# scraed/LanPaint

Measured on AMD Instinct MI355X. Metric: langevin_think_iterations_per_sec, higher is better.
Workload: dtype f32; 1 GPU; c2_sdxl: latent 1x4x128x128 per GPU, 30 sigmas x 5 think iterations, 50% box mask, stub backbone x->(0.9x,0.8x), VE/Karras schedule; rng=torch, graph=auto, mask_format=f32, mask_seen_by_kernels=bits, captured_calls=1, backbone_io=f32, replicas=1, rows_per_gpu=1, global_rows=1, latent_elements_per_gpu=65536

## Files before the change

lanpaint_amd/csrc/aux_kernels.hip:

```cpp
#include "lp_common.h"

namespace lp {

__global__ void lp_coeffs_kernel(lp_hyper h, const float* __restrict__ ve, int ve_stride,
                                 const float* __restrict__ abt, int abt_stride, const float* __restrict__ rs,
                                 int rs_stride, const float* __restrict__ step_ov, int step_stride,
                                 const float* __restrict__ t_model, int t_stride, int rows, float* __restrict__ table) {
    const int t = blockIdx.x * blockDim.x + threadIdx.x;
    const int r = t >> 2;
    if (r >= rows) return;
    const float abt_f = abt[static_cast<int64_t>(r) * abt_stride];
    const float ve_f = ve ? ve[static_cast<int64_t>(r) * ve_stride] : 0.0f;
    const float rs_f = rs ? rs[static_cast<int64_t>(r) * rs_stride] : 0.0f;
    const float tm_f = t_model ? t_model[static_cast<int64_t>(r) * t_stride] : 0.0f;
    const float oma = 1.0f - abt_f;
    const float step = step_ov ? step_ov[static_cast<int64_t>(r) * step_stride]
                               : h.step_size * fmaxf(oma, h.min_step_frac);
    coeffs_lane(h, abt_f, ve_f, rs_f, tm_f, step, (t >> 1) & 1, t & 1, table + static_cast<int64_t>(r) * LP_COEF_STRIDE);
}

__global__ void lp_sigma_times_kernel(const float* __restrict__ sigma, int rows, const float* __restrict__ schedule,
                                      int schedule_len, int is_flow, float* __restrict__ times,
                                      float* __restrict__ scalars, int32_t* __restrict__ seq_out, int32_t seq,
                                      const SigmaRule rule) {
    if (blockIdx.x != 0 || threadIdx.x >= kWave) return;
    sigma_rows_and_rule(sigma, rows, schedule, schedule_len, is_flow != 0, times, scalars, seq_out, seq, rule);
}

int sigma_times_rule_dispatch(const float* sigma, int rows, const float* schedule, int schedule_len, int is_flow,
                              float* times, float* scalars, int32_t* seq_out, int32_t seq, int32_t n_steps, int32_t early_stop,
                              int32_t total_steps, double min_step_frac, int32_t guess, uint64_t* valid_out, hipStream_t stream) {
    if (!sigma || !schedule || !times || !scalars || rows <= 0 || schedule_len <= 0) return LP_E_INVALID;
    const SigmaRule rule{n_steps, early_stop, total_steps, guess, min_step_frac, valid_out};
    hipLaunchKernelGGL(lp_sigma_times_kernel, dim3(1), dim3(64), 0, stream, sigma, rows, schedule, schedule_len, is_flow,
                       times, scalars, seq_out, seq, rule);
    return hipGetLastError() == hipSuccess ? LP_OK : LP_E_LAUNCH;
}

int sigma_times_dispatch(const float* sigma, int rows, const float* schedule, int schedule_len, int is_flow,
                         float* times, float* scalars, int32_t* seq_out, int32_t seq, hipStream_t stream) {
    return sigma_times_rule_dispatch(sigma, rows, schedule, schedule_len, is_flow, times, scalars, seq_out, seq, 0, 0, 0, 0.0, -1,
                                     nullptr, stream);
}

int coeffs_dispatch(const lp_hyper* h, const float* ve, int ve_stride, const float* abt, int abt_stride,
                    const float* rs, int rs_stride, const float* step_ov, int step_stride, const float* t_model,
                    int t_stride, int rows, float* table, hipStream_t stream) {
    if (!h || !abt || !table || rows <= 0) return LP_E_INVALID;
    if (!h->is_flow && !ve) return LP_E_INVALID;
    const int block = 64, lanes = rows * 4;
    hipLaunchKernelGGL(lp_coeffs_kernel, dim3((lanes + block - 1) / block), dim3(block), 0, stream, *h, ve, ve_stride,
                       abt, abt_stride, rs, rs_stride, step_ov, step_stride, t_model, t_stride, rows, table);
    return hipGetLastError() == hipSuccess ? LP_OK : LP_E_LAUNCH;
}

template <int VEC, int BLOCK>
__global__ __launch_bounds__(256) void lp_finalize_kernel(const void* a_mask, const void* a_model_out, const float* a_y,
                                                          const float* a_x_src, const uint64_t* a_io_table, int64_t a_n_el,
                                                          uint32_t a_flags, const lp_final_desc d_arg) {
    lp_final_desc d = d_arg;
    d.mask = a_mask; d.model_out = a_model_out; d.y = a_y; d.x_src = a_x_src; d.io_table = a_io_table;
    d.n_el = a_n_el; d.flags = a_flags;
    const int64_t groups = d.n_el / VEC;
    const int dt = x0_dtype(d.flags);
    const int64_t g = static_cast<int64_t>(blockIdx.x) * BLOCK + threadIdx.x;
    float* const x_dst = d.io_table ? reinterpret_cast<float*>(d.io_table[0]) : d.x_dst;
    float* const out = d.io_table ? reinterpret_cast<float*>(d.io_table[1]) : d.out;
    if (d.io_table && d.io_table[2] == 0ull) return;
    constexpr bool RA = VEC == 4 && BLOCK == 256;
    const bool in_range = g < groups;
    if (RA || in_range) {
        const int64_t i = (in_range ? g : groups - 1) * VEC;
        float m[VEC], mo[VEC], yv[VEC], o[VEC];
        Raw<VEC> m_raw, mo_raw, un_raw;
        load_mask_raw<VEC>(d.mask, d.flags, i, m_raw);
        float xs[VEC];
        bool need_mo = true, need_y = true;
        if constexpr (RA) {
            if (x_dst) load_f32<VEC>(d.x_src, i, xs);
            if ((d.flags & LP_FL_MASK_BITS) && !(d.flags & (LP_FL_CFG_FUSED | LP_FL_NO_REGION_SKIP))) {
                const uint32_t nib = (m_raw.w[0] >> (static_cast<uint32_t>(i) & 31u)) & 0xFu;
                need_y = __ballot(in_range && nib != 0u) != 0ull;
                need_mo = __ballot(in_range && nib != 0xFu) != 0ull;
            }
            if (!in_range) return;
        }
#pragma unroll
        for (int k = 0; k < VEC; ++k) mo_raw.w[k] = 0u, yv[k] = 0.0f;
        if (need_mo) load_raw<VEC>(d.model_out, dt, i, mo_raw);
        if (d.flags & LP_FL_CFG_FUSED) load_raw<VEC>(d.uncond, dt, i, un_raw);
        if (need_y) load_f32<VEC>(d.y, i, yv);
        if constexpr (!RA) {
            if (x_dst) load_f32<VEC>(d.x_src, i, xs);
        }
        cvt_mask<VEC>(d.flags, i, m_raw, m);
        cvt_raw<VEC>(dt, mo_raw, mo);
        if (d.flags & LP_FL_CFG_FUSED) {
            float un[VEC];
            cvt_raw<VEC>(dt, un_raw, un);
#pragma unroll
            for (int k = 0; k < VEC; ++k) mo[k] = un[k] + (mo[k] - un[k]) * d.cfg_scale;
        }
#pragma unroll
        for (int k = 0; k < VEC; ++k) o[k] = mo[k] * (1.0f - m[k]) + yv[k] * m[k];
        store_f32<VEC>(out, i, o);
        if (x_dst) store_f32<VEC>(x_dst, i, xs);
    }
    if (d.rng_bump_ptr && blockIdx.x == 0 && threadIdx.x == 0) *d.rng_bump_ptr += d.rng_bump;
}

static bool aligned(const void* p, size_t a) { return p == nullptr || (reinterpret_cast<uintptr_t>(p) % a) == 0; }

int finalize_dispatch(const lp_final_desc* dp, hipStream_t stream) {
    if (!dp) return LP_E_INVALID;
    const lp_final_desc& d = *dp;
    if (d.n_el <= 0 || !d.model_out || !d.y || !d.mask || (!d.out && !d.io_table)) return LP_E_INVALID;
    if ((d.x_dst || d.io_table) && !d.x_src) return LP_E_INVALID;
    if ((d.flags & LP_FL_CFG_FUSED) && !d.uncond) return LP_E_INVALID;
    if ((d.flags & LP_FL_MASK_BITS) && ((d.flags & (LP_FL_MASK_U8 | LP_FL_MASK_DENOISE)) || !aligned(d.mask, 4)))
        return LP_E_INVALID;
    const bool half = x0_dtype(d.flags) != DT_F32;
    const bool vec4 = (d.n_el % 4 == 0) && aligned(d.model_out, half ? 8 : 16) && aligned(d.uncond, half ? 8 : 16) &&
                      aligned(d.y, 16) &&
                      aligned(d.mask, (d.flags & (LP_FL_MASK_U8 | LP_FL_MASK_BITS)) ? 4 : 16) && aligned(d.x_src, 16) &&
                      (d.io_table ? true : (aligned(d.x_dst, 16) && aligned(d.out, 16)));
    const int vec = vec4 ? 4 : 1;
    const int64_t groups = d.n_el / vec;
    const int block = groups <= 64 * 1024 ? 64 : 256;
    const int64_t bx = (groups + block - 1) / block;
    if (bx > 0x7fffffff) return LP_E_INVALID;
#define LP_FINAL_ARGS d.mask, d.model_out, d.y, d.x_src, d.io_table, d.n_el, d.flags, d
    const dim3 grid(static_cast<unsigned>(bx));
    if (vec4 && block == 64) hipLaunchKernelGGL((lp_finalize_kernel<4, 64>), grid, dim3(64), 0, stream, LP_FINAL_ARGS);
    else if (vec4) hipLaunchKernelGGL((lp_finalize_kernel<4, 256>), grid, dim3(256), 0, stream, LP_FINAL_ARGS);
    else if (block == 64) hipLaunchKernelGGL((lp_finalize_kernel<1, 64>), grid, dim3(64), 0, stream, LP_FINAL_ARGS);
    else hipLaunchKernelGGL((lp_finalize_kernel<1, 256>), grid, dim3(256), 0, stream, LP_FINAL_ARGS);
#undef LP_FINAL_ARGS
    return hipGetLastError() == hipSuccess ? LP_OK : LP_E_LAUNCH;
}

__global__ __launch_bounds__(256) void lp_philox_kernel(float* __restrict__ out, int64_t n_el, uint64_t seed,
                                                        uint64_t offset, uint32_t slot) {
    for (int64_t e = static_cast<int64_t>(blockIdx.x) * blockDim.x + threadIdx.x; e < n_el;
         e += static_cast<int64_t>(gridDim.x) * blockDim.x) {
        float za, zb;
        normal_pair(static_cast<uint64_t>(e), offset, seed, za, zb);
        out[e] = slot ? zb : za;
    }
}

int philox_dispatch(float* out, int64_t n_el, uint64_t seed, uint64_t offset, uint32_t slot, hipStream_t stream) {
    if (!out || n_el <= 0) return LP_E_INVALID;
    if (slot > 1) return LP_E_INVALID;
    int64_t bx = (n_el + 255) / 256;
    if (bx > 4096) bx = 4096;
    hipLaunchKernelGGL(lp_philox_kernel, dim3(static_cast<unsigned>(bx)), dim3(256), 0, stream, out, n_el, seed,
                       offset, slot);
    return hipGetLastError() == hipSuccess ? LP_OK : LP_E_LAUNCH;
}

constexpr int kRingRows = 32, kRingCols = 62;

__global__ __launch_bounds__(256) void lp_ring_kernel(const float* __restrict__ mask, float* __restrict__ ring,
                                                      int height, int width) {
    __shared__ unsigned long long rowbits[kRingRows + 2];
    const int lane = threadIdx.x & (kWave - 1), wave = threadIdx.x / kWave;
    const int x0 = blockIdx.x * kRingCols - 1, y0 = blockIdx.y * kRingRows - 1;
    const int64_t plane = static_cast<int64_t>(blockIdx.z) * height * width;
    const int x = x0 + lane;
    const bool x_in = x >= 0 && x < width;

    for (int j = wave; j < kRingRows + 2; j += 4) {
        const int y = y0 + j;
        bool known = false;
        if (x_in && y >= 0 && y < height) known = mask[plane + static_cast<int64_t>(y) * width + x] > 0.5f;
        const unsigned long long bits = __ballot(known);
        if (lane == 0) rowbits[j] = bits;
    }
    __syncthreads();
    for (int j = 1 + wave; j <= kRingRows; j += 4) {
        const int y = y0 + j;
        if (y >= height) break;
        const unsigned long long k = rowbits[j];
        const unsigned long long nb = (k << 1) | (k >> 1) | rowbits[j - 1] | rowbits[j + 1];
        const unsigned long long rb = ~k & nb;
        if (lane >= 1 && lane <= kRingCols && x_in) {
            const int64_t idx = plane + static_cast<int64_t>(y) * width + x;
            ring[idx] = ((rb >> lane) & 1ull) ? (1.0f - mask[idx]) : 0.0f;
        }
    }
}

int ring_dispatch(const float* mask, float* ring, int64_t planes, int height, int width, hipStream_t stream) {
    if (!mask || !ring || planes <= 0 || height <= 0 || width <= 0) return LP_E_INVALID;
    if (planes > 65535) return LP_E_UNSUPPORTED;
    dim3 grid((width + kRingCols - 1) / kRingCols, (height + kRingRows - 1) / kRingRows, static_cast<unsigned>(planes));
    if (grid.y > 65535) return LP_E_UNSUPPORTED;
    hipLaunchKernelGGL(lp_ring_kernel, grid, dim3(256), 0, stream, mask, ring, height, width);
    return hipGetLastError() == hipSuccess ? LP_OK : LP_E_LAUNCH;
}

template <int V>
__global__ __launch_bounds__(256) void lp_wmse_partial_kernel(const float* __restrict__ a, const float* __restrict__ b,
                                                              const float* __restrict__ mask,
                                                              const float* __restrict__ ring, int64_t n_el,
                                                              double* __restrict__ scratch) {
    __shared__ double part[4][4];
    float s[4] = {0.f, 0.f, 0.f, 0.f};
    const int64_t groups = n_el / V;
    for (int64_t g = static_cast<int64_t>(blockIdx.x) * blockDim.x + threadIdx.x; g < groups;
         g += static_cast<int64_t>(gridDim.x) * blockDim.x) {
        float av[V], bv[V], mv[V], rv[V];
        load_f32<V>(a, g * V, av);
        load_f32<V>(b, g * V, bv);
        load_f32<V>(mask, g * V, mv);
        if (ring) load_f32<V>(ring, g * V, rv);
#pragma unroll
        for (int k = 0; k < V; ++k) {
            const float dv = av[k] - bv[k];
            const float d2 = dv * dv;
            const float w1 = 1.0f - mv[k];
            s[0] += d2 * w1;
            s[1] += w1;
            if (ring) {
                s[2] += d2 * rv[k];
                s[3] += rv[k];
            }
        }
    }
    double v[4] = {static_cast<double>(s[0]), static_cast<double>(s[1]), static_cast<double>(s[2]), static_cast<double>(s[3])};
    wave_sum_dpp(v);
    const int lane = threadIdx.x & (kWave - 1), wave = threadIdx.x / kWave;
    if (lane == kWave - 1) {
#pragma unroll
        for (int k = 0; k < 4; ++k) part[wave][k] = v[k];
    }
    __syncthreads();
    if (threadIdx.x < 4) {
        const int k = threadIdx.x;
        scratch[static_cast<int64_t>(blockIdx.x) * 4 + k] = part[0][k] + part[1][k] + part[2][k] + part[3][k];
    }
}

__global__ __launch_bounds__(64) void lp_wmse_final_kernel(const double* __restrict__ scratch, int blocks, double* __restrict__ acc) {
    double v[4] = {0.0, 0.0, 0.0, 0.0};
    for (int bidx = threadIdx.x; bidx < blocks; bidx += kWave) {
#pragma unroll
        for (int k = 0; k < 4; ++k) v[k] += scratch[static_cast<int64_t>(bidx) * 4 + k];
    }
    wave_sum_dpp(v);
    if (threadIdx.x == kWave - 1) {
#pragma unroll
        for (int k = 0; k < 4; ++k) acc[k] = v[k];
    }
}

int wmse_dispatch(const float* a, const float* b, const float* mask, const float* ring, int64_t n_el, double* acc,
                  double* scratch, int scratch_blocks, hipStream_t stream) {
    if (!a || !b || !mask || !acc || !scratch || n_el <= 0 || scratch_blocks <= 0) return LP_E_INVALID;
    const auto al16 = [](const void* p) { return (reinterpret_cast<uintptr_t>(p) & 15u) == 0; };
    const bool vec4 = n_el % 4 == 0 && al16(a) && al16(b) && al16(mask) && (!ring || al16(ring));
// ... 110 lines not shown
```

lanpaint_amd/csrc/lp_common.h:

```cpp
#pragma once
#include <hip/hip_runtime.h>
#include <hip/hip_ext.h>
#include <stdint.h>

#include "lanpaint_hip.h"

namespace lp {

constexpr int kWave = 64;

__device__ __forceinline__ int nearest_exact_index(int i, int in_size, int out_size, int rule) {
#pragma clang fp contract(off)
    const float scale = static_cast<float>(in_size) / static_cast<float>(out_size);
    const float at = static_cast<float>(i) + 0.5f;
    int s;
    if (rule == LP_NN_ATEN_SCALAR) {
        s = static_cast<int>(floorf(at * scale));
    } else {
        float src = (rule == LP_NN_ATEN_CPU_GENERIC_FMA) ? __builtin_fmaf(scale, at, -0.5f) : (scale * at - 0.5f);
        src = src < 0.0f ? 0.0f : src;
        s = static_cast<int>(floorf(static_cast<float>(static_cast<double>(src) + 0.5)));
    }
    return s < in_size - 1 ? s : in_size - 1;
}
// ... 241 lines not shown
            const u2 t = __builtin_nontemporal_load(reinterpret_cast<const u2*>(q));
            r.w[0] = t.x; r.w[1] = t.y;
        } else {
#pragma unroll
            for (int k = 0; k < V; ++k) r.w[k] = q[k];
        }
    }
}



template <int V>
__device__ __forceinline__ void cvt_raw(int dt, const Raw<V>& r, float (&o)[V]) {
    if (dt == DT_F32) {
#pragma unroll
        for (int k = 0; k < V; ++k) o[k] = __uint_as_float(r.w[k]);
    } else {
        uint16_t h[V];
        if constexpr (V == 4) {
            h[0] = r.w[0] & 0xffffu; h[1] = r.w[0] >> 16; h[2] = r.w[1] & 0xffffu; h[3] = r.w[1] >> 16;
        } else {
#pragma unroll
            for (int k = 0; k < V; ++k) h[k] = static_cast<uint16_t>(r.w[k]);
        }
#pragma unroll
        for (int k = 0; k < V; ++k) o[k] = (dt == DT_BF16) ? bf16_to_f32(h[k]) : f16_to_f32(h[k]);
    }
}

template <int V>
__device__ __forceinline__ void cvt_raw(int dt, const Raw<V>& r, float (&o)[V], int64_t) {
    cvt_raw<V>(dt, r, o);
}

template <int V, int W, typename IX>
__device__ __forceinline__ void load_raw_w(const void* __restrict__ p, int dt, const IX& i, Raw<V>& r) {
    if constexpr (W == 4) load_raw<V>(p, DT_F32, i, r);
    else if constexpr (W == 2) load_raw<V>(p, DT_BF16, i, r);
    else load_raw<V>(p, dt, i, r);
}

template <int V>
__device__ __forceinline__ void load_any(const void* __restrict__ p, int dt, int64_t i, float (&o)[V]) {
    Raw<V> r;
    load_raw<V>(p, dt, i, r);
    cvt_raw<V>(dt, r, o);
}


template <int V>
__device__ __forceinline__ void store_any(void* __restrict__ p, int dt, int64_t i, const float (&v)[V]) {
    if (dt == DT_F32) {
        store_f32<V>(static_cast<float*>(p), i, v);
    } else {
        uint16_t* q = static_cast<uint16_t*>(p) + i;
        if constexpr (V == 4) {
            u2 t;
            t.x = pack_half2(dt, v[0], v[1]); t.y = pack_half2(dt, v[2], v[3]);
            __builtin_nontemporal_store(t, reinterpret_cast<u2*>(q));
        } else {
#pragma unroll
            for (int k = 0; k < V; ++k) q[k] = (dt == DT_BF16) ? f32_to_bf16(v[k]) : f32_to_f16(v[k]);
        }
    }
}

typedef uint32_t u4 __attribute__((ext_vector_type(4)));
template <int CTRL>
__device__ __forceinline__ uint32_t dpp_quad(uint32_t v) {
    return static_cast<uint32_t>(__builtin_amdgcn_update_dpp(0, static_cast<int>(v), CTRL, 0xf, 0xf, false));
}

__device__ __forceinline__ void load_raw_pair(const void* __restrict__ p, int64_t i, bool pair_on, Raw<4>& r) {
    if ((threadIdx.x & 1u) == 0u && pair_on) {
        const u4 t = __builtin_nontemporal_load(reinterpret_cast<const u4*>(static_cast<const uint16_t*>(p) + i));
        r.w[0] = t.x; r.w[1] = t.y; r.w[2] = t.z; r.w[3] = t.w;
    }
}

__device__ __forceinline__ void cvt_raw_pair(int dt, const Raw<4>& r, float (&o)[4]) {
    const uint32_t hi0 = dpp_quad<0xA0>(r.w[2]), hi1 = dpp_quad<0xA0>(r.w[3]);
    const bool odd = (threadIdx.x & 1u) != 0u;
    const uint32_t w0 = odd ? hi0 : r.w[0], w1 = odd ? hi1 : r.w[1];
    const uint16_t h[4] = {static_cast<uint16_t>(w0 & 0xffffu), static_cast<uint16_t>(w0 >> 16),
                           static_cast<uint16_t>(w1 & 0xffffu), static_cast<uint16_t>(w1 >> 16)};
#pragma unroll
    for (int k = 0; k < 4; ++k) o[k] = (dt == DT_BF16) ? bf16_to_f32(h[k]) : f16_to_f32(h[k]);
}

__device__ __forceinline__ void store_half_pair(void* __restrict__ p, int dt, int64_t i, const float (&v)[4]) {
    const uint32_t w0 = pack_half2(dt, v[0], v[1]), w1 = pack_half2(dt, v[2], v[3]);
    const uint32_t p0 = dpp_quad<0xF5>(w0), p1 = dpp_quad<0xF5>(w1);
    if ((threadIdx.x & 1u) == 0u) {
        const u4 t = {w0, w1, p0, p1};
        __builtin_nontemporal_store(t, reinterpret_cast<u4*>(static_cast<uint16_t*>(p) + i));
    }
}

template <int V>
__device__ __forceinline__ void load_mask_raw(const void* __restrict__ p, uint32_t flags, int64_t i, Raw<V>& r) {
    if (flags & LP_FL_MASK_BITS) {
        r.w[0] = static_cast<const uint32_t*>(p)[i >> 5];
    } else if (flags & LP_FL_MASK_U8) {
        const uint8_t* q = static_cast<const uint8_t*>(p) + i;
        if constexpr (V == 4) {
            r.w[0] = *reinterpret_cast<const uint32_t*>(q);
        } else {
#pragma unroll
            for (int k = 0; k < V; ++k) r.w[k] = q[k];
        }
    } else {
        float t[V];
        load_f32<V>(static_cast<const float*>(p), i, t);
#pragma unroll
        for (int k = 0; k < V; ++k) r.w[k] = __float_as_uint(t[k]);
    }
}



template <int V>
__device__ __forceinline__ void cvt_mask(uint32_t flags, int64_t i, const Raw<V>& r, float (&m)[V]) {
    if (flags & LP_FL_MASK_BITS) {
        const uint32_t sh = static_cast<uint32_t>(i) & 31u;
#pragma unroll
        for (int k = 0; k < V; ++k) m[k] = static_cast<float>((r.w[0] >> (sh + k)) & 1u);
        return;
    }
    if (flags & LP_FL_MASK_U8) {
#pragma unroll
        for (int k = 0; k < V; ++k) m[k] = static_cast<float>(V == 4 ? ((r.w[0] >> (8 * k)) & 0xffu) : r.w[k]);
    } else {
#pragma unroll
        for (int k = 0; k < V; ++k) m[k] = __uint_as_float(r.w[k]);
    }
    if (flags & LP_FL_MASK_DENOISE) {
#pragma unroll
        for (int k = 0; k < V; ++k) m[k] = 1.0f - ((m[k] > 0.5f) ? 1.0f : 0.0f);
    }
}

template <int V>
__device__ __forceinline__ void load_mask(const void* __restrict__ p, uint32_t flags, int64_t i, float (&m)[V]) {
    Raw<V> r;
    load_mask_raw<V>(p, flags, i, r);
    cvt_mask<V>(flags, i, r, m);
}

__device__ __forceinline__ float row_scale(bool flow, float abt_f, float ve_f) {
#pragma clang fp contract(off)
    return flow ? (sqrtf(abt_f) + sqrtf(1.0f - abt_f)) : sqrtf(1.0f + ve_f * ve_f);
}

__device__ inline void coeffs_lane(const lp_hyper& h, float abt_f, float ve_f, float rs_f, float tm_f, float step,
                                   int g, int s, float* __restrict__ c) {
#pragma clang fp contract(off)
    const float oma = 1.0f - abt_f;
    const float dtx2 = 2.0f * step * 1.0f, dty2 = 2.0f * step * h.beta;
    const float dtx = dtx2 / 2.0f, dty = dty2 / 2.0f;
    if (g == 0 && s == 0) {
        const float atx = (1.0f / oma) * dtx2 / 2.0f;
        const float aty = (h.one_plus_lambda / oma) * dty2 / 2.0f;
        const bool valid = step > 0.0f;
        c[LP_C_SCALE] = row_scale(h.is_flow, abt_f, ve_f);
        c[LP_C_SQRT_ABT] = sqrtf(abt_f);
        c[LP_C_OMA] = oma;
        c[LP_C_ABT] = abt_f;
        c[LP_C_RSIGMA] = rs_f;
        c[LP_C_DTX] = dtx;
        c[LP_C_DTY] = dty;
        c[LP_C_AX] = atx / dtx;
        c[LP_C_AY] = aty / dty;
        c[LP_C_DX] = sqrtf(2.0f);
        c[LP_C_DY] = sqrtf(2.0f);
        c[LP_C_VALID] = valid ? 1.0f : 0.0f;
        c[LP_C_TMODEL] = tm_f;
        c[LP_C_RSCALE] = static_cast<float>(1.0 / static_cast<double>(c[LP_C_SCALE]));
    }
    const double oma_d = static_cast<double>(oma);
    float* q = c + (g ? LP_C_REGION1 : LP_C_REGION0);
    const double a = (g ? static_cast<double>(h.one_plus_lambda) : 1.0) / oma_d;
    const double dt = static_cast<double>(g ? dty : dtx);
    const double tau = s ? dt * 0.5 : dt;
    const double e = exp(-a * tau);
    const double k = -expm1(-a * tau) / a;
    const double k2 = -expm1(-2.0 * a * tau) / (2.0 * a);
    const double sd = sqrt(fmax(2.0 * k2, 0.0));
    q[s ? LP_R_E_HALF : LP_R_E_FULL] = static_cast<float>(e);
    q[s ? LP_R_K_HALF : LP_R_K_FULL] = static_cast<float>(k);
    q[s ? LP_R_STD_HALF : LP_R_STD_FULL] = static_cast<float>(sd);
    if (s == 0) {
        const double cx0 = sqrt(static_cast<double>(abt_f)) / oma_d;
        q[LP_R_DT] = static_cast<float>(dt);
        q[LP_R_A] = static_cast<float>(a);
        q[LP_R_CX0] = static_cast<float>(cx0);
        q[LP_R_CXT] = g ? static_cast<float>(a - 1.0 / oma_d) : 0.0f;
    }
}

__device__ __forceinline__ double wave_sum(double v) {
#pragma unroll
    for (int off = kWave / 2; off > 0; off >>= 1) v += __shfl_down(v, off, kWave);
    return v;
}

template <int CTRL, int ROW_MASK>
__device__ __forceinline__ float dpp_move(float v) {
    return __builtin_bit_cast(float, __builtin_amdgcn_update_dpp(0, __builtin_bit_cast(int, v), CTRL, ROW_MASK, 0xf, false));
}
template <int CTRL, int ROW_MASK>
__device__ __forceinline__ double dpp_move(double v) {
    const long long b = __builtin_bit_cast(long long, v);
    const int lo = __builtin_amdgcn_update_dpp(0, static_cast<int>(b), CTRL, ROW_MASK, 0xf, false);
    const int hi = __builtin_amdgcn_update_dpp(0, static_cast<int>(b >> 32), CTRL, ROW_MASK, 0xf, false);
    return __builtin_bit_cast(double, (static_cast<long long>(hi) << 32) | static_cast<long long>(static_cast<uint32_t>(lo)));
}
template <int CTRL, int ROW_MASK, typename T, int N>
__device__ __forceinline__ void dpp_level(T (&v)[N]) {
    T t[N];
#pragma unroll
    for (int k = 0; k < N; ++k) t[k] = dpp_move<CTRL, ROW_MASK>(v[k]);
#pragma unroll
    for (int k = 0; k < N; ++k) v[k] += t[k];
}
template <typename T, int N>
__device__ __forceinline__ void wave_sum_dpp(T (&v)[N]) {
    dpp_level<0xb1, 0xf>(v);
    dpp_level<0x4e, 0xf>(v);
    dpp_level<0x124, 0xf>(v);
    dpp_level<0x128, 0xf>(v);
    dpp_level<0x142, 0xa>(v);
    dpp_level<0x143, 0xc>(v);
}

__device__ __forceinline__ void sigma_to_times(float s, bool is_flow, float& ve, float& abt, float& ft) {
#pragma clang fp contract(off)
    if (is_flow) {
        const float a = 1.0f - s;
        const float a2 = a * a;
        const float s2 = s * s;
        const float den = a2 + s2;
        abt = a2 / den;
        ve = s / a;
        ft = s;
    } else {
        ve = s;
        const float s2 = s * s;
        const float den = 1.0f + s2;
        abt = 1.0f / den;
        const float b = 1.0f - abt;
        const float sb = sqrtf(b), sa = sqrtf(abt);
        const float sden = sb + sa;
        ft = sb / sden;
    }
}

struct SigmaRule {
    int32_t n_steps, early_stop, total_steps, guess;
    double min_step_frac;
    uint64_t* valid_out;
};

__host__ __device__ inline int32_t effective_inner_steps(int32_t n_steps, double step_f, double frac, int32_t total_steps,
                                                         int32_t early_stop, double min_step_frac);

__device__ __forceinline__ void sigma_rows_and_rule(const float* __restrict__ sigma, int rows, const float* __restrict__ schedule,
                                                    int schedule_len, bool is_flow, float* __restrict__ times,
                                                    float* __restrict__ scalars, int32_t* __restrict__ seq_out, int32_t seq,
                                                    const SigmaRule& rule) {
#pragma clang fp contract(off)
    const int lane = static_cast<int>(threadIdx.x) & (kWave - 1);
    float sum_sigma = 0.0f, sum_oma = 0.0f;
    for (int r0 = 0; r0 < rows; r0 += kWave) {
        const int r = r0 + lane;
        float s = 0.0f, oma = 0.0f;
        if (r < rows) {
            s = sigma[r];
            float ve, abt, ft;
            sigma_to_times(s, is_flow, ve, abt, ft);
            if (times) {
                times[r] = ve;
                times[rows + r] = abt;
                times[2 * rows + r] = ft;
            }
            oma = 1.0f - abt;
        }
        const int n = rows - r0 < kWave ? rows - r0 : kWave;
        for (int k = 0; k < n; ++k) {
            sum_sigma = sum_sigma + __builtin_bit_cast(float, __builtin_amdgcn_readlane(__builtin_bit_cast(int, s), k));
            sum_oma = sum_oma + __builtin_bit_cast(float, __builtin_amdgcn_readlane(__builtin_bit_cast(int, oma), k));
        }
    }
    const float mean_sigma = sum_sigma / static_cast<float>(rows);
    int best = 0;
    float best_d = INFINITY;
    for (int i = lane; i < schedule_len; i += kWave) {
        const float diff = schedule[i] - mean_sigma;
        const float dd = fabsf(diff);
        if (dd < best_d) {
            best_d = dd;
            best = i;
        }
    }
#pragma unroll
    for (int off = 1; off < kWave; off <<= 1) {
        const float od = __shfl_xor(best_d, off, kWave);
        const int ob = __shfl_xor(best, off, kWave);
        if (od < best_d || (od == best_d && ob < best)) {
            best_d = od;
            best = ob;
        }
    }
    if (lane != 0) return;
    const float frac = sum_oma / static_cast<float>(rows);
    scalars[0] = static_cast<float>(best);
    scalars[1] = frac;
    if (rule.valid_out) {
        const int32_t n_eff = effective_inner_steps(rule.n_steps, static_cast<double>(static_cast<float>(best)),
                                                    static_cast<double>(frac), rule.total_steps, rule.early_stop,
                                                    rule.min_step_frac);
        *rule.valid_out = (rule.guess < 0 || rule.guess == n_eff) ? 1ull : 0ull;
        scalars[3] = static_cast<float>(n_eff);
    }
    if (seq_out) {
        __threadfence_system();
        __hip_atomic_store(seq_out, seq, __ATOMIC_RELEASE, __HIP_MEMORY_SCOPE_SYSTEM);
    }
}

__host__ __device__ inline int32_t effective_inner_steps(int32_t n_steps, double step_f, double frac, int32_t total_steps,
                                                         int32_t early_stop, double min_step_frac) {
    if (total_steps - static_cast<int32_t>(step_f) <= early_stop) return 0;
    if (min_step_frac <= 0.0 || frac >= min_step_frac || n_steps <= 0) return n_steps;
    const double r = rint(static_cast<double>(n_steps) * frac / min_step_frac);
    return r > 0.0 ? static_cast<int32_t>(r) : 0;
}

__host__ __device__ inline int x0_dtype(uint32_t flags) {
    return (flags & LP_FL_X0_BF16) ? DT_BF16 : (flags & LP_FL_X0_F16) ? DT_F16 : DT_F32;
}
__host__ __device__ inline int xin_dtype(uint32_t flags) {
    return (flags & LP_FL_XIN_BF16) ? DT_BF16 : (flags & LP_FL_XIN_F16) ? DT_F16 : DT_F32;
}

struct StepPlan {
    const void* kernel;
    dim3 grid;
    uint32_t ph_ct;
    int vec;
    bool decide;
// ... 18 lines not shown
```

lanpaint_amd/csrc/step_kernel.hip:

```cpp
#include <cstddef>

#include "lp_common.h"

#pragma clang fp contract(off)

namespace lp {

struct RegionCoef {
    float e_full, k_full, std_full, e_half, k_half, std_half, dt, a, cx0, cxt;
};

struct RowCoef {
    float scale, sqrt_abt, oma, abt, rsigma, dtx, dty, ax, ay, dx, dy, valid;
    RegionCoef reg[2];
    float rscale;
};

__device__ __forceinline__ RowCoef load_row(const float* __restrict__ coef, int row) {
    const float* c = coef + static_cast<int64_t>(row) * LP_COEF_STRIDE;
    RowCoef r;
    r.scale = c[LP_C_SCALE]; r.sqrt_abt = c[LP_C_SQRT_ABT]; r.oma = c[LP_C_OMA]; r.abt = c[LP_C_ABT];
    r.rsigma = c[LP_C_RSIGMA]; r.dtx = c[LP_C_DTX]; r.dty = c[LP_C_DTY]; r.ax = c[LP_C_AX]; r.ay = c[LP_C_AY];
    r.dx = c[LP_C_DX]; r.dy = c[LP_C_DY]; r.valid = c[LP_C_VALID];
    r.rscale = c[LP_C_RSCALE];
// ... 271 lines not shown
    lp_step_desc d = d_arg;
    d.x_t = static_cast<float*>(a0); d.C = static_cast<float*>(a1);
    if constexpr ((PH & LP_PH_REPLACE) != 0) {
        d.x = static_cast<const float*>(a2);
        d.known = d.noise = static_cast<const float*>(a3);
        d.y = static_cast<const float*>(a4); d.mask = a5;
    } else {
        d.x0 = a2; d.x0_big = a3;
        if constexpr (SMALL) {
            d.coef = static_cast<const float*>(a4); d.rng_offset_ptr = static_cast<const uint64_t*>(a5);
        } else {
            d.y = static_cast<const float*>(a4); d.mask = a5;
        }
    }
    d.el_per_row = a_el_per_row; d.flags = a_flags;
    static_assert(!ES || (!ST && !PER_EL && (PH & LP_PH_REPLACE) == 0), "early stop: think-step launches of the row-table modes");
    constexpr bool es_fold = ES == 2;
    int row = blockIdx.y;
    int64_t st_base = 0, st_lo = 0, st_hi = 0;
    uint32_t st_round = 0;
    if constexpr (ST) {
        const int64_t span = 4 * static_cast<int64_t>(d.rng_bg), epr = d.el_per_row;
        const uint32_t rounds = d.rng_inc >> 2, per_round = gridDim.y / rounds;
        st_round = blockIdx.y / per_round;
        st_base = static_cast<int64_t>(st_round) * span;
        row = static_cast<int>(st_base / epr) + static_cast<int>(blockIdx.y - st_round * per_round);
        const int64_t row_lo = static_cast<int64_t>(row) * epr, row_hi = row_lo + epr;
        st_lo = row_lo > st_base ? row_lo : st_base;
        st_hi = row_hi < st_base + span ? row_hi : st_base + span;
        if (row >= d.rows || st_lo >= st_hi) return;
        const int64_t i0 = st_base + static_cast<int64_t>(blockIdx.x) * kBlock, i1 = i0 + kBlock;
        bool any = false;
#pragma unroll
        for (int k = 0; k < 4; ++k) {
            const int64_t s0 = i0 + k * static_cast<int64_t>(d.rng_bg), s1 = i1 + k * static_cast<int64_t>(d.rng_bg);
            any = any || (s0 < st_hi && s1 > st_lo);
        }
        if (!any) return;
    }
    const uint32_t fl = d.flags;
    bool es_gated = false, es_idle = false;
    int es_prev = -1, es_anchor = -1, es_write = 0;
    bool es_keeper = false;
    lp_es_state es_lite;
    uint2 es_words[8];
    double es_fv[kEsSums];
    if constexpr (ES) {
        es_gated = (fl & LP_FL_ES_GATED) != 0;
        if constexpr (es_fold) {
            const int rd = (d.es_index + 1) & 1;
            const lp_es_state* sp = d.es + rd;
            if constexpr (VEC == 4) {
                const uint2* sv = reinterpret_cast<const uint2*>(sp);
#pragma unroll
                for (int k = 0; k < 8; ++k) es_words[k] = sv[k];
            } else {
                uint32_t lane_zero;
                asm volatile("v_mov_b32 %0, 0" : "=v"(lane_zero));
                const uint2* sv = reinterpret_cast<const uint2*>(sp) + lane_zero;
#pragma unroll
                for (int k = 0; k < 8; ++k) es_words[k] = sv[k];
            }
            es_keeper = blockIdx.x == 0 && blockIdx.y == 0 && threadIdx.x == 0;
            if constexpr (VEC != 4) {
                if (threadIdx.x < kWave) {
                    const double* src = es_acc_set(d, d.es_index - 1) + static_cast<size_t>(threadIdx.x) * 8;
#pragma unroll
                    for (int k = 0; k < kEsSums; ++k) es_fv[k] = src[k];
                }
            }
        } else {
            es_prev = d.es->cur_slot; es_anchor = d.es->anchor_slot; es_write = d.es->write_slot;
            if (es_gated && d.es->stopped != 0) {
                const int64_t g = static_cast<int64_t>(blockIdx.x) * kBlock + threadIdx.x;
                if (g >= d.el_per_row / VEC) return;
                const int64_t i = static_cast<int64_t>(row) * d.el_per_row + g * VEC;
                float xt[VEC], xo[VEC];
                load_f32<VEC>(d.x_t, i, xt);
                if constexpr (PH == 0 && MODE == MODE_ROW && !ST) {
                    if (fl & LP_FL_AV) {
                        const uint32_t word = static_cast<const uint32_t*>(d.av_bits)[i >> 5];
                        const uint32_t nib = word >> (static_cast<uint32_t>(i) & 31u);
#pragma unroll
                        for (int k = 0; k < VEC; ++k) {
                            const float sc = d.coef[static_cast<int64_t>(2 * row + static_cast<int>((nib >> k) & 1u)) * LP_COEF_STRIDE + LP_C_SCALE];
                            xo[k] = (fl & LP_FL_FLOW) ? xt[k] / sc : xt[k] * sc;
                        }
                        store_any<VEC>(d.x_in, xin_dtype(fl), i, xo);
                        return;
                    }
                }
                const float sc = load_row(d.coef, row).scale;
#pragma unroll
                for (int k = 0; k < VEC; ++k) xo[k] = (fl & LP_FL_FLOW) ? xt[k] / sc : xt[k] * sc;
                store_any<VEC>(d.x_in, xin_dtype(fl), i, xo);
                return;
            }
        }
    }
    const uint32_t ph = PH ? PH : d.phases;
    const bool flow = fl & LP_FL_FLOW;
    const bool post = ph & kPost;
    constexpr bool HOT = PH != 0 && ES == 0 && (RNG == 0 || (RNG == 1 && VEC == 1));
    constexpr bool TS = HOT && RNG == 1 && VEC == 1;
    static_assert(!TS || (!ST && (PH & LP_PH_REPLACE) == 0), "TS: think launches only");
    const bool given = HOT ? false : (fl & LP_FL_X0S_GIVEN) != 0;
    const int x0dt = X0W == 4 ? static_cast<int>(DT_F32) : x0_dtype(fl), xindt = xin_dtype(fl);
    const int64_t groups = ST ? static_cast<int64_t>(d.rng_bg) : d.el_per_row / VEC;
    const int64_t row_base = static_cast<int64_t>(row) * d.el_per_row;
    const float lam = d.lambda, opl = d.one_plus_lambda;

    RowCoef rc;
    bool av_mixed = false;
    uint32_t av_nib = 0u;
    const bool fold_coeffs = (ph & LP_PH_COEFFS) != 0;
    constexpr bool fold_sigma = (PH & LP_PH_SIGMA) != 0;
    static_assert(!fold_sigma || PH != 0, "LP_PH_SIGMA: the phase-specialised kernels only");
    auto row_times = [&](float& abt_f, float& ve_f, float& rs_f, float& tm_f) __attribute__((always_inline)) {
        if constexpr (fold_sigma) {
            float ft;
            rs_f = d.sg_sigma[row];
            sigma_to_times(rs_f, flow, ve_f, abt_f, ft);
            tm_f = flow ? ft : ve_f;
        } else {
            abt_f = d.t_abt[static_cast<int64_t>(row) * d.t_abt_stride];
            ve_f = d.t_ve ? d.t_ve[static_cast<int64_t>(row) * d.t_ve_stride] : 0.0f;
            rs_f = d.t_rsig ? d.t_rsig[static_cast<int64_t>(row) * d.t_rsig_stride] : 0.0f;
            tm_f = 0.0f;
        }
    };
    if (fold_coeffs) {
        auto build_table = [&](float abt_f, float ve_f, float rs_f, float tm_sig) __attribute__((always_inline)) {
            if (threadIdx.x < 4) {
                lp_hyper h;
                h.lambda = d.lambda; h.beta = d.beta; h.step_size = d.step_size; h.min_step_frac = d.min_step_frac;
                h.is_flow = flow ? 1 : 0; h.one_plus_lambda = d.one_plus_lambda;
                const float tm_f = fold_sigma ? tm_sig : (d.t_model ? d.t_model[static_cast<int64_t>(row) * d.t_model_stride] : 0.0f);
                const float step = d.step_size * fmaxf(1.0f - abt_f, d.min_step_frac);
                coeffs_lane(h, abt_f, ve_f, rs_f, tm_f, step, (threadIdx.x >> 1) & 1, threadIdx.x & 1,
                            d.coef_out + static_cast<int64_t>(row) * LP_COEF_STRIDE);
                if (row == 0 && threadIdx.x == 0 && d.rng_state_out) {
                    d.rng_state_out[0] = d.rng_state_val[0];
                    d.rng_state_out[1] = d.rng_state_val[1];
                }
            }
        };
        auto sigma_rule = [&]() __attribute__((always_inline)) {
            const SigmaRule rule{d.sg_n_steps, d.sg_early_stop, d.sg_total_steps, d.sg_guess, d.sg_min_step_frac, d.sg_valid_out};
            sigma_rows_and_rule(d.sg_sigma, d.rows, d.sg_schedule, d.sg_schedule_len, flow, d.sg_times_out,
                                d.sg_scalars_out, d.sg_seq_out, d.sg_seq, rule);
        };
        if constexpr (TBL) {
            if (blockIdx.x == 0) {
                if (threadIdx.x < kWave) {
                    float abt_f, ve_f, rs_f, tm_f;
                    row_times(abt_f, ve_f, rs_f, tm_f);
                    build_table(abt_f, ve_f, rs_f, tm_f);
                    LP_CLK(5)
                } else if (fold_sigma && blockIdx.y == 0 && threadIdx.x < 2 * kWave) {
                    sigma_rule();
                }
                LP_CLK(6)
                LP_CLK_FLUSH
                return;
            }
        } else {
            float abt_f, ve_f, rs_f, tm_f;
            row_times(abt_f, ve_f, rs_f, tm_f);
            if constexpr (fold_sigma) {
                if (blockIdx.x == 0 && blockIdx.y == 0 && threadIdx.x < kWave) sigma_rule();
            }
            if (blockIdx.x == 0) build_table(abt_f, ve_f, rs_f, tm_f);
            rc.scale = row_scale(flow, abt_f, ve_f);
            rc.rscale = 1.0f / rc.scale;
            rc.rsigma = rs_f;
        }
    } else {
        if constexpr (PH == 0) {
            if ((ph & LP_PH_REPLACE) && d.rng_state_out && blockIdx.x == 0 && blockIdx.y == 0 && threadIdx.x == 0) {
                d.rng_state_out[0] = d.rng_state_val[0];
                d.rng_state_out[1] = d.rng_state_val[1];
            }
        }
        if constexpr (!PER_EL) {
            if constexpr (SMALL && PH != 0) {
                static_assert(VEC == 1, "load_row_early leaves rc.rscale poisoned: the div_shared paths (VEC == 4) must use load_row");
                rc = load_row_early(d.coef, row);
            } else {
                int crow = row;
                if constexpr (PH == 0 && MODE == MODE_ROW && !ST) {
                    if (fl & LP_FL_AV) {
                        const int64_t g0 = static_cast<int64_t>(blockIdx.x) * kBlock + threadIdx.x;
                        const bool in_row = g0 < groups;
                        const int64_t i0 = row_base + (in_row ? g0 : groups - 1) * VEC;
                        const uint32_t word = static_cast<const uint32_t*>(d.av_bits)[i0 >> 5];
                        av_nib = (word >> (static_cast<uint32_t>(i0) & 31u)) & ((1u << VEC) - 1u);
                        const bool any_audio = __ballot(in_row && av_nib != 0u) != 0ull;
                        const bool any_video = __ballot(in_row && av_nib != ((1u << VEC) - 1u)) != 0ull;
                        av_mixed = any_audio && any_video;
                        crow = 2 * row + ((any_audio && !any_video) ? 1 : 0);
                    }
                }
                rc = load_row(d.coef, crow);
            }
        }
    }

    uint64_t rng_w0 = 0, rng_w1 = 0;
    bool rng_have = false;
    if constexpr (TS) {
        typedef const __attribute__((address_space(4))) uint64_t* state_words;
        rng_have = d.rng_offset_ptr != nullptr;
        const state_words sw = (state_words)(rng_have ? d.rng_offset_ptr : reinterpret_cast<const uint64_t*>(d.coef));
        const uint64_t w0 = sw[0], w1 = sw[1];
        rng_w0 = rng_have ? w0 : 0ull;
        rng_w1 = rng_have ? w1 : 0ull;
    } else if constexpr (SMALL) {
        if (d.rng_offset_ptr) {
            rng_w0 = d.rng_offset_ptr[0];
            rng_w1 = d.rng_offset_ptr[1];
            rng_have = true;
        }
    }

    const int64_t g_raw = static_cast<int64_t>(el_bx) * kBlock + threadIdx.x;
    int64_t st_i = 0;
    if constexpr (ST) st_i = st_base + static_cast<int64_t>(threadIdx.x >> 6) * static_cast<int64_t>(d.rng_bg) +
                             static_cast<int64_t>(blockIdx.x) * kBlock + static_cast<int64_t>(threadIdx.x & 63) * VEC;
    const bool active = ST ? (st_i >= st_lo && st_i < st_hi) : (g_raw < groups);
    if constexpr (!ES && !ST) {
        if (!active) return;
    }
    const int64_t g = active ? g_raw : groups - 1;
    float es_p[kEsSums] = {0.f, 0.f, 0.f, 0.f, 0.f, 0.f};
    bool es_zero_wave = false;
    {
        const int64_t i = ST ? (active ? st_i : st_lo) : row_base + g * VEC;

        constexpr bool AVK = PH == 0 && MODE == MODE_ROW && !ST;
        auto av_row = [&](int k) __attribute__((always_inline)) -> const float* {
            return d.coef + static_cast<int64_t>(2 * row + static_cast<int>((av_nib >> k) & 1u)) * LP_COEF_STRIDE;
        };
        auto av_ld = [&](const float* c, int f) __attribute__((always_inline)) -> float {
            return __hip_atomic_load(c + f, __ATOMIC_RELAXED, __HIP_MEMORY_SCOPE_WAVEFRONT);
        };
        auto row_scale_of = [&](int k) __attribute__((always_inline)) -> float {
            if constexpr (AVK) {
                if (av_mixed) return av_ld(av_row(k), LP_C_SCALE);
            }
            return rc.scale;
        };
        auto row_rsigma_of = [&](int k) __attribute__((always_inline)) -> float {
            if constexpr (AVK) {
                if (av_mixed) return av_ld(av_row(k), LP_C_RSIGMA);
            }
            return rc.rsigma;
        };
        auto elem_of = [&](int k, float mk) __attribute__((always_inline)) -> ElemCoef {
            float ax = rc.ax, ay = rc.ay, dx = rc.dx, dy = rc.dy, dtx = rc.dtx, dty = rc.dty, sq = rc.sqrt_abt, oma = rc.oma,
                  sc = rc.scale, valid = rc.valid;
            if constexpr (AVK) {
                if (av_mixed) {
                    const float* c = av_row(k);
                    ax = av_ld(c, LP_C_AX); ay = av_ld(c, LP_C_AY); dx = av_ld(c, LP_C_DX); dy = av_ld(c, LP_C_DY);
                    dtx = av_ld(c, LP_C_DTX); dty = av_ld(c, LP_C_DTY); sq = av_ld(c, LP_C_SQRT_ABT); oma = av_ld(c, LP_C_OMA);
                    sc = av_ld(c, LP_C_SCALE); valid = av_ld(c, LP_C_VALID);
                }
            }
            const float om = 1.0f - mk;
            ElemCoef e;
            e.a = ax * om + ay * mk;
            e.d = dx * om + dy * mk;
            e.dt = dtx * om + dty * mk;
            e.sqrt_abt = sq;
            e.oma = oma;
            e.scale = sc;
            e.valid = valid != 0.0f;
            return e;
        };

        auto form_verdict = [&]() __attribute__((always_inline)) {
                const int it = d.es_index;
                {
                    const auto u = [&](int w) { return __builtin_amdgcn_readfirstlane(static_cast<int>((w & 1) ? es_words[w >> 1].y : es_words[w >> 1].x)); };
                    const auto u64 = [&](int w) { return (static_cast<uint64_t>(static_cast<uint32_t>(u(w + 1))) << 32) | static_cast<uint32_t>(u(w)); };
                    static_assert(offsetof(lp_es_state, enabled) == 28 && offsetof(lp_es_state, seq_base) == 32 &&
                                  offsetof(lp_es_state, abt_val) == 56, "lp_es_state layout");
                    es_lite.stopped = u(0); es_lite.counter = u(1); es_lite.n_ran = u(2); es_lite.cur_slot = u(3);
                    es_lite.anchor_slot = u(4); es_lite.write_slot = u(5); es_lite.enabled = u(7);
                    es_lite.seq_base = static_cast<int64_t>(u64(8)); es_lite.total_ran = static_cast<int64_t>(u64(10));
                    es_lite.threshold_eff = __longlong_as_double(static_cast<long long>(u64(12)));
                    es_lite.abt_val = __longlong_as_double(static_cast<long long>(u64(14)));
                }
                int v_stopped = 0, v_cur = -1, v_anchor = -1, v_write = 0;
                bool v_have = false;
                if (it > 0 && es_lite.stopped == 0) {
                    __shared__ int fold_out[4];
                    if (threadIdx.x < kWave) {
                        float tot[kEsSums];
                        if constexpr (VEC == 4) {
                            const double* src = es_acc_set(d, d.es_index - 1) + static_cast<size_t>(threadIdx.x) * 8;
#pragma unroll
                            for (int k = 0; k < kEsSums; ++k) es_fv[k] = src[k];
                        }
                        if constexpr (VEC != 4) {
#pragma unroll
                            for (int k = 0; k < kEsSums; ++k) asm volatile("" : "+v"(es_fv[k]));
                        }
                        es_slot_total(es_fv, tot);
                        const bool hp = es_lite.cur_slot >= 0, ha = es_lite.anchor_slot >= 0;
                        es_decide(d, es_lite, tot, hp, ha, it - 1, es_keeper);
                        if (threadIdx.x == 0) {
                            fold_out[0] = es_lite.stopped; fold_out[1] = es_lite.cur_slot;
// ... 973 lines not shown
```

Before: 125,400 think-iterations/s.

## Split coefficient table build across waves and hoist finalize table loads

The coefficient table build in the step kernel's block 0 is split so that different waves compute the exp, expm1 and sqrt double-precision pieces (and the header) in parallel, instead of one wave doing all of them serially. The finalize kernel now reads the io_table words through the constant address space up front, defers the early-exit and output pointer resolution until after the data loads, and reads the RNG counter early so that its latency overlaps the loads. The aim is to shorten the latency-bound critical path of these small kernels. This adds complexity, and it assumes that at least four waves per block exist for the table build.

```diff
diff --git a/lanpaint_amd/csrc/aux_kernels.hip b/lanpaint_amd/csrc/aux_kernels.hip
--- a/lanpaint_amd/csrc/aux_kernels.hip
+++ b/lanpaint_amd/csrc/aux_kernels.hip
@@ -61,52 +61,62 @@
     lp_final_desc d = d_arg;
     d.mask = a_mask; d.model_out = a_model_out; d.y = a_y; d.x_src = a_x_src; d.io_table = a_io_table;
     d.n_el = a_n_el; d.flags = a_flags;
+    typedef const __attribute__((address_space(4))) uint64_t* table_words;
+    const bool have_table = d.io_table != nullptr;
+    const table_words tw = have_table ? (table_words)d.io_table
+                                      : (table_words)__builtin_amdgcn_kernarg_segment_ptr();
+    const uint64_t tw0 = tw[0], tw1 = tw[1], tw2 = tw[2];
     const int64_t groups = d.n_el / VEC;
     const int dt = x0_dtype(d.flags);
     const int64_t g = static_cast<int64_t>(blockIdx.x) * BLOCK + threadIdx.x;
-    float* const x_dst = d.io_table ? reinterpret_cast<float*>(d.io_table[0]) : d.x_dst;
-    float* const out = d.io_table ? reinterpret_cast<float*>(d.io_table[1]) : d.out;
-    if (d.io_table && d.io_table[2] == 0ull) return;
     constexpr bool RA = VEC == 4 && BLOCK == 256;
     const bool in_range = g < groups;
-    if (RA || in_range) {
-        const int64_t i = (in_range ? g : groups - 1) * VEC;
-        float m[VEC], mo[VEC], yv[VEC], o[VEC];
-        Raw<VEC> m_raw, mo_raw, un_raw;
-        load_mask_raw<VEC>(d.mask, d.flags, i, m_raw);
-        float xs[VEC];
-        bool need_mo = true, need_y = true;
-        if constexpr (RA) {
-            if (x_dst) load_f32<VEC>(d.x_src, i, xs);
-            if ((d.flags & LP_FL_MASK_BITS) && !(d.flags & (LP_FL_CFG_FUSED | LP_FL_NO_REGION_SKIP))) {
-                const uint32_t nib = (m_raw.w[0] >> (static_cast<uint32_t>(i) & 31u)) & 0xFu;
-                need_y = __ballot(in_range && nib != 0u) != 0ull;
-                need_mo = __ballot(in_range && nib != 0xFu) != 0ull;
-            }
-            if (!in_range) return;
+    if (!RA && !in_range) return;
+    const bool want_xs = BLOCK == 64 ? d.x_src != nullptr : (have_table || d.x_dst != nullptr);
+    const int64_t i = (in_range ? g : groups - 1) * VEC;
+    float m[VEC], mo[VEC], yv[VEC], o[VEC];
+    Raw<VEC> m_raw, mo_raw, un_raw;
+    load_mask_raw<VEC>(d.mask, d.flags, i, m_raw);
+    float xs[VEC];
+    bool need_mo = true, need_y = true;
+    if constexpr (RA) {
+        if (want_xs) load_f32<VEC>(d.x_src, i, xs);
+        if ((d.flags & LP_FL_MASK_BITS) && !(d.flags & (LP_FL_CFG_FUSED | LP_FL_NO_REGION_SKIP))) {
+            const uint32_t nib = (m_raw.w[0] >> (static_cast<uint32_t>(i) & 31u)) & 0xFu;
+            need_y = __ballot(in_range && nib != 0u) != 0ull;
+            need_mo = __ballot(in_range && nib != 0xFu) != 0ull;
         }
-#pragma unroll
-        for (int k = 0; k < VEC; ++k) mo_raw.w[k] = 0u, yv[k] = 0.0f;
-        if (need_mo) load_raw<VEC>(d.model_out, dt, i, mo_raw);
-        if (d.flags & LP_FL_CFG_FUSED) load_raw<VEC>(d.uncond, dt, i, un_raw);
-        if (need_y) load_f32<VEC>(d.y, i, yv);
-        if constexpr (!RA) {
-            if (x_dst) load_f32<VEC>(d.x_src, i, xs);
-        }
-        cvt_mask<VEC>(d.flags, i, m_raw, m);
-        cvt_raw<VEC>(dt, mo_raw, mo);
-        if (d.flags & LP_FL_CFG_FUSED) {
-            float un[VEC];
-            cvt_raw<VEC>(dt, un_raw, un);
-#pragma unroll
-            for (int k = 0; k < VEC; ++k) mo[k] = un[k] + (mo[k] - un[k]) * d.cfg_scale;
-        }
-#pragma unroll
-        for (int k = 0; k < VEC; ++k) o[k] = mo[k] * (1.0f - m[k]) + yv[k] * m[k];
-        store_f32<VEC>(out, i, o);
-        if (x_dst) store_f32<VEC>(x_dst, i, xs);
-    }
-    if (d.rng_bump_ptr && blockIdx.x == 0 && threadIdx.x == 0) *d.rng_bump_ptr += d.rng_bump;
+        if (!in_range) return;
+    }
+#pragma unroll
+    for (int k = 0; k < VEC; ++k) mo_raw.w[k] = 0u, yv[k] = 0.0f;
+    if (need_mo) load_raw<VEC>(d.model_out, dt, i, mo_raw);
+    if (d.flags & LP_FL_CFG_FUSED) load_raw<VEC>(d.uncond, dt, i, un_raw);
+    if (need_y) load_f32<VEC>(d.y, i, yv);
+    if constexpr (!RA) {
+        if (want_xs) load_f32<VEC>(d.x_src, i, xs);
+    }
+    asm volatile("" ::"s"(tw0), "s"(tw1), "s"(tw2), "s"(d.x_dst), "s"(d.out), "s"(d.rng_bump_ptr), "s"(d.rng_bump),
+                 "s"(d.uncond), "s"(__float_as_uint(d.cfg_scale)));
+    const bool bumper = d.rng_bump_ptr != nullptr && blockIdx.x == 0 && threadIdx.x == 0;
+    uint64_t counter = 0;
+    if (bumper) counter = *d.rng_bump_ptr;
+    cvt_mask<VEC>(d.flags, i, m_raw, m);
+    cvt_raw<VEC>(dt, mo_raw, mo);
+    if (d.flags & LP_FL_CFG_FUSED) {
+        float un[VEC];
+        cvt_raw<VEC>(dt, un_raw, un);
+#pragma unroll
+        for (int k = 0; k < VEC; ++k) mo[k] = un[k] + (mo[k] - un[k]) * d.cfg_scale;
+    }
+#pragma unroll
+    for (int k = 0; k < VEC; ++k) o[k] = mo[k] * (1.0f - m[k]) + yv[k] * m[k];
+    if (have_table && tw2 == 0ull) return;
+    float* const x_dst = have_table ? reinterpret_cast<float*>(tw0) : d.x_dst;
+    float* const out = have_table ? reinterpret_cast<float*>(tw1) : d.out;
+    store_f32<VEC>(out, i, o);
+    if (x_dst) store_f32<VEC>(x_dst, i, xs);
+    if (bumper) *d.rng_bump_ptr = counter + d.rng_bump;
 }
 
 static bool aligned(const void* p, size_t a) { return p == nullptr || (reinterpret_cast<uintptr_t>(p) % a) == 0; }
diff --git a/lanpaint_amd/csrc/lp_common.h b/lanpaint_amd/csrc/lp_common.h
--- a/lanpaint_amd/csrc/lp_common.h
+++ b/lanpaint_amd/csrc/lp_common.h
@@ -417,12 +417,16 @@
     return flow ? (sqrtf(abt_f) + sqrtf(1.0f - abt_f)) : sqrtf(1.0f + ve_f * ve_f);
 }
 
-__device__ inline void coeffs_lane(const lp_hyper& h, float abt_f, float ve_f, float rs_f, float tm_f, float step,
-                                   int g, int s, float* __restrict__ c) {
+enum : unsigned { LP_CP_HEADER = 1u, LP_CP_E = 2u, LP_CP_K = 4u, LP_CP_SD = 8u, LP_CP_TAIL = 16u, LP_CP_ALL = 31u };
+
+template <unsigned P>
+__device__ __forceinline__ void coeffs_pieces(const lp_hyper& h, float abt_f, float ve_f, float rs_f, float tm_f, float step,
+                                              int g, int s, float* __restrict__ c) {
 #pragma clang fp contract(off)
     const float oma = 1.0f - abt_f;
     const float dtx2 = 2.0f * step * 1.0f, dty2 = 2.0f * step * h.beta;
     const float dtx = dtx2 / 2.0f, dty = dty2 / 2.0f;
+    if constexpr ((P & LP_CP_HEADER) != 0) {
     if (g == 0 && s == 0) {
         const float atx = (1.0f / oma) * dtx2 / 2.0f;
         const float aty = (h.one_plus_lambda / oma) * dty2 / 2.0f;
@@ -442,18 +446,24 @@
         c[LP_C_TMODEL] = tm_f;
         c[LP_C_RSCALE] = static_cast<float>(1.0 / static_cast<double>(c[LP_C_SCALE]));
     }
+    }
+    if constexpr ((P & ~LP_CP_HEADER) == 0) return;
     const double oma_d = static_cast<double>(oma);
     float* q = c + (g ? LP_C_REGION1 : LP_C_REGION0);
     const double a = (g ? static_cast<double>(h.one_plus_lambda) : 1.0) / oma_d;
     const double dt = static_cast<double>(g ? dty : dtx);
     const double tau = s ? dt * 0.5 : dt;
-    const double e = exp(-a * tau);
-    const double k = -expm1(-a * tau) / a;
-    const double k2 = -expm1(-2.0 * a * tau) / (2.0 * a);
-    const double sd = sqrt(fmax(2.0 * k2, 0.0));
-    q[s ? LP_R_E_HALF : LP_R_E_FULL] = static_cast<float>(e);
-    q[s ? LP_R_K_HALF : LP_R_K_FULL] = static_cast<float>(k);
-    q[s ? LP_R_STD_HALF : LP_R_STD_FULL] = static_cast<float>(sd);
+    double e, k, sd;
+    if constexpr ((P & LP_CP_E) != 0) e = exp(-a * tau);
+    if constexpr ((P & LP_CP_K) != 0) k = -expm1(-a * tau) / a;
+    if constexpr ((P & LP_CP_SD) != 0) {
+        const double k2 = -expm1(-2.0 * a * tau) / (2.0 * a);
+        sd = sqrt(fmax(2.0 * k2, 0.0));
+    }
+    if constexpr ((P & LP_CP_E) != 0) q[s ? LP_R_E_HALF : LP_R_E_FULL] = static_cast<float>(e);
+    if constexpr ((P & LP_CP_K) != 0) q[s ? LP_R_K_HALF : LP_R_K_FULL] = static_cast<float>(k);
+    if constexpr ((P & LP_CP_SD) != 0) q[s ? LP_R_STD_HALF : LP_R_STD_FULL] = static_cast<float>(sd);
+    if constexpr ((P & LP_CP_TAIL) != 0) {
     if (s == 0) {
         const double cx0 = sqrt(static_cast<double>(abt_f)) / oma_d;
         q[LP_R_DT] = static_cast<float>(dt);
@@ -461,6 +471,12 @@
         q[LP_R_CX0] = static_cast<float>(cx0);
         q[LP_R_CXT] = g ? static_cast<float>(a - 1.0 / oma_d) : 0.0f;
     }
+    }
+}
+
+__device__ inline void coeffs_lane(const lp_hyper& h, float abt_f, float ve_f, float rs_f, float tm_f, float step,
+                                   int g, int s, float* __restrict__ c) {
+    coeffs_pieces<LP_CP_ALL>(h, abt_f, ve_f, rs_f, tm_f, step, g, s, c);
 }
 
 __device__ __forceinline__ double wave_sum(double v) {
diff --git a/lanpaint_amd/csrc/step_kernel.hip b/lanpaint_amd/csrc/step_kernel.hip
--- a/lanpaint_amd/csrc/step_kernel.hip
+++ b/lanpaint_amd/csrc/step_kernel.hip
@@ -447,13 +447,35 @@
         };
         if constexpr (TBL) {
             if (blockIdx.x == 0) {
-                if (threadIdx.x < kWave) {
-                    float abt_f, ve_f, rs_f, tm_f;
-                    row_times(abt_f, ve_f, rs_f, tm_f);
-                    build_table(abt_f, ve_f, rs_f, tm_f);
+                const unsigned wave = threadIdx.x / kWave, lane = threadIdx.x & (kWave - 1);
+                const bool rule_wave = fold_sigma && blockIdx.y == 0;
+                if (rule_wave && wave == 1) {
+                    sigma_rule();
+                } else if (lane < 4) {
+                    float abt_f, ve_f, rs_f, tm_sig;
+                    row_times(abt_f, ve_f, rs_f, tm_sig);
+                    lp_hyper h;
+                    h.lambda = d.lambda; h.beta = d.beta; h.step_size = d.step_size; h.min_step_frac = d.min_step_frac;
+                    h.is_flow = flow ? 1 : 0; h.one_plus_lambda = d.one_plus_lambda;
+                    const float step = d.step_size * fmaxf(1.0f - abt_f, d.min_step_frac);
+                    const int g = (lane >> 1) & 1, s = lane & 1;
+                    float* const c = d.coef_out + static_cast<int64_t>(row) * LP_COEF_STRIDE;
+                    if (wave == 0) {
+                        if (row == 0 && lane == 0 && d.rng_state_out) {
+                            d.rng_state_out[0] = d.rng_state_val[0];
+                            d.rng_state_out[1] = d.rng_state_val[1];
+                        }
+                        coeffs_pieces<LP_CP_SD>(h, abt_f, ve_f, rs_f, 0.0f, step, g, s, c);
+                    } else if (wave == 2) {
+                        coeffs_pieces<LP_CP_K>(h, abt_f, ve_f, rs_f, 0.0f, step, g, s, c);
+                    } else if (wave == 3) {
+                        coeffs_pieces<LP_CP_E | LP_CP_TAIL>(h, abt_f, ve_f, rs_f, 0.0f, step, g, s, c);
+                    }
+                    if (wave == (rule_wave ? 2u : 1u) && lane == 0) {
+                        const float tm_f = fold_sigma ? tm_sig : (d.t_model ? d.t_model[static_cast<int64_t>(row) * d.t_model_stride] : 0.0f);
+                        coeffs_pieces<LP_CP_HEADER>(h, abt_f, ve_f, rs_f, tm_f, step, 0, 0, c);
+                    }
                     LP_CLK(5)
-                } else if (fold_sigma && blockIdx.y == 0 && threadIdx.x < 2 * kWave) {
-                    sigma_rule();
                 }
                 LP_CLK(6)
                 LP_CLK_FLUSH
```

Result: no change. 126,400 think-iterations/s, median of 6 (+0.8%).
